# jacobwulffwold/GAN_SR_wind_field

Hardware: AMD Instinct MI355X
Metric: GAN train-steps/sec (G+D fwd+bwd) (higher is better)
Workload: dtype bf16; 1 GPU; C3' full G+D adversarial step: LR 32x32x128 -> HR 128x128x128 (x4), batch 1/GPU, G 16 RRDB nf128 (34.77M), D bf32; preset=C3p, global_batch=1, parallelism=dp1, ranks=1

## Files before the change

### gan_sr_wind_field_amd/csrc/conv_wgrad_tile.hip

```cpp
#include <cstdlib>

#include "common.h"

namespace {

typedef __attribute__((ext_vector_type(4))) short s16x4_t;
typedef s16x4_t __attribute__((address_space(3))) * lds_s16x4_ptr;

struct WgtArgs {
  const unsigned short* x;
  const unsigned short* x2;
  int x2_ctot, x2_c0;
  const unsigned short* dy;
  float* dw;
  const void* zero16;
  int B, Xi, Yi, Zi, Xo, Yo, Zo;
  int Cin, in_ctot, in_off;
  int Cout, out_ctot, out_off;
  int KX, KY, KZ, px, py, pz, ups;
  int TX, TY, TZ;
  int n_chunks, c_chunks, S;
  int tiles_x, tiles_y, tiles_z, ntiles;
  int nbuf;
  int xp_bytes;
  int xs_bytes, buf_bytes;
  int off_buf;
  int tri_base, tri_step;
  int n_active;
  unsigned char act_nc[64], act_cc[64];
  long part_stride;
  int yl_m, yl_ox, yl_oy;
  int xl_m, xl_ox, xl_oy;
  int xl_mz, xl_oz;
  int prio;
  int nphase;
  long class_stride;
  float* bias_parts;
  int S_forced;
  int plan_only;
  unsigned long long* stamps;
  int ablate;
};

__device__ __forceinline__ uint4 tr_frag(const char* lo, const char* hi) {
  s16x4_t a = __builtin_amdgcn_ds_read_tr16_b64_v4i16((lds_s16x4_ptr)(lo));
  s16x4_t b = __builtin_amdgcn_ds_read_tr16_b64_v4i16((lds_s16x4_ptr)(hi));
  uint2 l2 = __builtin_bit_cast(uint2, a), h2 = __builtin_bit_cast(uint2, b);
  return make_uint4(l2.x, l2.y, h2.x, h2.y);
}

__device__ __forceinline__ void glds16(const void* gsrc, unsigned lds_addr) {
  unsigned keep;
  asm volatile(
      "s_mov_b32 %0, m0\n\ts_mov_b32 m0, %2\n\ts_nop 0\n\tglobal_load_lds_dwordx4 %1, off\n\ts_mov_b32 m0, %0"
      : "=&s"(keep)
      : "v"(gsrc), "s"(lds_addr)
      : "memory");
}
__device__ __forceinline__ void dma_wait() { asm volatile("s_waitcnt vmcnt(0)" ::: "memory"); }
__device__ __forceinline__ void dma_wait_upto(int n) {
#define WG_VM(k) case k: asm volatile("s_waitcnt vmcnt(" #k ")" ::: "memory"); break;
  switch (n) {
    WG_VM(0) WG_VM(1) WG_VM(2) WG_VM(3) WG_VM(4) WG_VM(5) WG_VM(6) WG_VM(7) WG_VM(8) WG_VM(9) WG_VM(10) WG_VM(11)
    WG_VM(12) WG_VM(13) WG_VM(14) WG_VM(15) WG_VM(16) WG_VM(17) WG_VM(18) WG_VM(19) WG_VM(20) WG_VM(21) WG_VM(22)
    WG_VM(23) WG_VM(24) WG_VM(25) WG_VM(26) WG_VM(27) WG_VM(28) WG_VM(29) WG_VM(30) WG_VM(31) WG_VM(32) WG_VM(33)
    default: asm volatile("s_waitcnt vmcnt(0)" ::: "memory");
  }
#undef WG_VM
}

#ifdef WSR_CT_STAMPS
#define WG_STAMP(k)                                                                                    \
  do {                                                                                                 \
    if (a.stamps && threadIdx.x == 0) a.stamps[(size_t)blockIdx.x * 8 + (k)] = (k) >= 6 ? clock64() : wall_clock64(); \
  } while (0)
#else
#define WG_STAMP(k) do {} while (0)
#endif

template <int TN> __device__ __forceinline__ int ysw(int v) { return TN == 1 ? 0 : (TN <= 4 ? (v >> 1) & 3 : v & 7); }
constexpr int wgt_rby(int tn) { return tn == 1 ? 32 : (tn <= 4 ? 128 : 256); }

constexpr int wgt_xk(int spw, int tn) { return spw * tn * 4 >= 192 ? 5 : 6; }
constexpr int wgt_yk(int spw, int tn) { return spw * tn * 4 >= 192 ? 4 : 5; }

template <int TN, int SPW, int CT, bool Z16, bool BIAS>
__device__ __forceinline__ void wgrad_tile_body(const WgtArgs& a) {
  static_assert(!BIAS || (TN == 8 && SPW == 1), "one n-tile per wave");
  constexpr int WAVES = 8, NT = 512;
  constexpr int XRPU = 32;
  constexpr int XK = wgt_xk(SPW, TN), YK = wgt_yk(SPW, TN);
  constexpr int RBY = wgt_rby(TN);
  constexpr int YRPU = 1024 / RBY;
  static_assert(TN <= 8, "dy rows hold at most 128 channels");
  extern __shared__ __attribute__((aligned(16))) char smem[];
  const int t = threadIdx.x, lane = t & 63;
  const int wave = __builtin_amdgcn_readfirstlane(t >> 6);
  WG_STAMP(0);
  WG_STAMP(6);

  const int Ly = a.TY + a.KY - 1, Lz = a.TZ + a.KZ - 1, Lx = a.TX + a.KX - 1;
  const int L = Lx * Ly * Lz;
  const int M = a.TX * a.TY * a.TZ;
  const int taps = a.KX * a.KY * a.KZ;
  unsigned short* htab = reinterpret_cast<unsigned short*>(smem);
  char* buf0 = smem + a.off_buf;
  typedef __attribute__((address_space(3))) char* lptr_t;
  const unsigned buf_lds = (unsigned)(unsigned long)(lptr_t)buf0;

  int bid = xcd_remap(blockIdx.x, gridDim.x);
  int cc, nc, s0;
  int cls = 0;
  if (a.nphase == 4) {
    cls = bid & 3;
    bid >>= 2;
  }
  const int px = a.px - (cls >> 1), py = a.py - (cls & 1);
  const int yl_ox = a.nphase == 4 ? (a.yl_m == 2 ? cls >> 1 : 0) : a.yl_ox;
  const int yl_oy = a.nphase == 4 ? (a.yl_m == 2 ? cls & 1 : 0) : a.yl_oy;
  const int xl_ox = a.nphase == 4 ? (a.xl_m == 2 ? px : 0) : a.xl_ox;
  const int xl_oy = a.nphase == 4 ? (a.xl_m == 2 ? py : 0) : a.xl_oy;
  if (a.n_active > 0) {
    const int pr = bid % a.n_active;
    s0 = bid / a.n_active;
    cc = a.act_cc[pr];
    nc = a.act_nc[pr];
  } else {
    cc = bid % a.c_chunks;
    bid /= a.c_chunks;
    nc = bid % a.n_chunks;
    s0 = bid / a.n_chunks;
  }
  const int c0 = cc * 16 * CT, n0 = nc * 16 * TN;
  const bool second = a.x2 != nullptr && c0 >= a.x2_c0;
  const unsigned short* xt = second ? a.x2 : a.x;
  const int x_ctot = second ? a.x2_ctot : a.in_ctot;
  const int x_off = second ? c0 - a.x2_c0 : a.in_off + c0;

  bool act[TN];
  bool any = false;
#pragma unroll
  for (int i = 0; i < TN; ++i) {
    const int n = n0 + 16 * i;
    bool ok = n < a.Cout;
    if (ok && a.tri_step > 0) {
      const int n_last = (n + 15 < a.Cout) ? n + 15 : a.Cout - 1;
      ok = c0 < a.tri_base + a.tri_step * (n_last / a.tri_step);
    }
    act[i] = ok;
    any = any || ok;
  }
  if (!any) return;

  for (int m = t; m < M; m += NT) {
    const int oz = m % a.TZ, r = m / a.TZ;
    const int oy = r % a.TY, ox = r / a.TY;
    htab[m] = (unsigned short)((ox * Ly + oy) * Lz + oz);
  }

  const int U = a.ups ? 1 : 0;
  const int parx = U ? ((-px) & 1) : 0, pary = U ? ((-py) & 1) : 0;
  const int XUP = (L + XRPU - 1) / XRPU;
  const int XU = XUP * CT;
  const int YU = (M + YRPU - 1) / YRPU;
  unsigned xgeo[XK], ygeo[YK];
  int xrel[XK], yrel[YK];
#pragma unroll
  for (int k = 0; k < XK; ++k) {
    const int u = wave + WAVES * k;
    unsigned geo = 0;
    int rel = 0;
    if (u < XU) {
      const int ct = u / XUP;
      const int h = (u - ct * XUP) * XRPU + (lane >> 1);
      const int ch8 = 2 * ct + (lane & 1);
      if (h < L && c0 + 8 * ch8 < a.Cin) {
        const int hz = h % Lz, qq = h / Lz;
        const int hy = qq % Ly, hx = qq / Ly;
        geo = hx | (hy << 8) | (hz << 16) | (1u << 24);
        rel = ((((hx + parx) >> U) * a.xl_m * (a.Yi * a.xl_m) + ((hy + pary) >> U) * a.xl_m) * (a.Zi * a.xl_mz) +
               hz * a.xl_mz) * x_ctot + 8 * ch8;
      }
    }
    xgeo[k] = geo;
    xrel[k] = rel;
  }
#pragma unroll
  for (int k = 0; k < YK; ++k) {
    const int u = wave + WAVES * k;
    unsigned geo = 0;
    int rel = 0;
    if (u < YU) {
      const int v = u * YRPU + lane / (RBY / 16), sl = lane % (RBY / 16);
      const int b32 = (sl >> 1) ^ ysw<TN>(v);
      const int oct = 2 * b32 + (sl & 1);
      if (v < M && b32 < TN && n0 + 8 * oct < a.Cout) {
        const int oz = v % a.TZ, qq = v / a.TZ;
        const int oy = qq % a.TY, ox = qq / a.TY;
        geo = ox | (oy << 8) | (oz << 16) | (1u << 24);
        rel = ((ox * a.yl_m * (a.Yo * a.yl_m) + oy * a.yl_m) * a.Zo + oz) * a.out_ctot + 8 * oct;
      }
    }
    ygeo[k] = geo;
    yrel[k] = rel;
  }

  const unsigned short* zsrc = reinterpret_cast<const unsigned short*>(a.zero16);
  auto issue_tile = [&](int tile, int buf) {
    int r = tile;
    const int tz = r % a.tiles_z; r /= a.tiles_z;
    const int ty = r % a.tiles_y; r /= a.tiles_y;
    const int tx = r % a.tiles_x;
    const int b = r / a.tiles_x;
    const int x0 = tx * a.TX, y0 = ty * a.TY, z0 = tz * a.TZ;
    const unsigned dstx = buf_lds + buf * a.buf_bytes;
    const unsigned dsty = dstx + a.xs_bytes;
    {
      const int lox = px - x0, loy = py - y0, loz = a.pz - z0;
      const int sx_ = a.Xi << U, sy_ = a.Yi << U;
      const bool inner = lox <= 0 && Lx - lox <= sx_ && loy <= 0 && Ly - loy <= sy_ && loz <= 0 && Lz - loz <= a.Zi;
      const long base = ((((long)b * a.Xi * a.xl_m + (long)((x0 - px - parx) >> U) * a.xl_m + xl_ox) * (a.Yi * a.xl_m) +
                          (long)((y0 - py - pary) >> U) * a.xl_m + xl_oy) * (a.Zi * a.xl_mz) +
                         (long)(z0 - a.pz) * a.xl_mz + a.xl_oz) * x_ctot + x_off;
      const unsigned short* bp = xt + base;
#pragma unroll
      for (int k = 0; k < XK; ++k) {
        const int u = wave + WAVES * k;
#ifdef WSR_CT_STAMPS
        if ((a.ablate & 64) && (k & 1)) continue;
        if ((a.ablate & 128) && (k & 3)) continue;
#endif
        if (u < XU) {
          const unsigned geo = xgeo[k];
          bool ok = (geo >> 24) & 1;
          if (!inner)
            ok = ok && (unsigned)((int)(geo & 255) - lox) < (unsigned)sx_ &&
                 (unsigned)((int)((geo >> 8) & 255) - loy) < (unsigned)sy_ &&
                 (unsigned)((int)((geo >> 16) & 255) - loz) < (unsigned)a.Zi;
          glds16(ok ? bp + xrel[k] : zsrc, __builtin_amdgcn_readfirstlane(dstx + u * 1024));
        }
      }
    }
    {
      const int hix = a.Xo - x0, hiy = a.Yo - y0, hiz = a.Zo - z0;
      const bool inner = a.TX <= hix && a.TY <= hiy && a.TZ <= hiz;
      const long base = ((((long)b * a.Xo * a.yl_m + x0 * a.yl_m + yl_ox) * (a.Yo * a.yl_m) + y0 * a.yl_m + yl_oy) *
                             a.Zo + z0) * a.out_ctot + a.out_off + n0;
      const unsigned short* bp = a.dy + base;
#pragma unroll
      for (int k = 0; k < YK; ++k) {
        const int u = wave + WAVES * k;
        if (u < YU) {
          const unsigned geo = ygeo[k];
          bool ok = (geo >> 24) & 1;
          if (!inner)
            ok = ok && (int)(geo & 255) < hix && (int)((geo >> 8) & 255) < hiy && (int)((geo >> 16) & 255) < hiz;
          glds16(ok ? bp + yrel[k] : zsrc, __builtin_amdgcn_readfirstlane(dsty + u * 1024));
        }
      }
    }
  };

  const int nslots = taps * CT;
  int soff[SPW];
#pragma unroll
  for (int j = 0; j < SPW; ++j) {
    const int sj = wave + WAVES * j;
    int off = 0, ct = 0;
    if (sj < nslots) {
      const int tap = sj / CT;
      ct = sj % CT;
      const int kz = tap % a.KZ, r = tap / a.KZ;
      const int ky = r % a.KY, kx = r / a.KY;
      off = (kx * Ly + ky) * Lz + kz;
    }
    soff[j] = __builtin_amdgcn_readfirstlane(off * 32 + ct * a.xp_bytes);
  }

  f32x4_t acc[SPW][TN];
#pragma unroll
  for (int j = 0; j < SPW; ++j)
#pragma unroll
    for (int i = 0; i < TN; ++i) acc[j][i] = f32x4_t{0.f, 0.f, 0.f, 0.f};
  f32x4_t accb = f32x4_t{0.f, 0.f, 0.f, 0.f};

  const int G = lane >> 4, q = (lane & 15) >> 2, p = lane & 3;
  const int ksteps = M >> 5;

  WG_STAMP(1);
#ifdef WSR_CT_STAMPS
  long long st_bar = 0;
  int st_tiles = 0;
#endif
  constexpr bool LEAN = SPW * TN * 4 >= 192;
  constexpr int R = SPW % 7 == 0 ? 7 : (SPW % 4 == 0 ? 4 : (SPW % 3 == 0 ? 3 : 1));
#ifdef WSR_WG_D
  constexpr int D = R > WSR_WG_D ? WSR_WG_D : R - 1;
#else
  constexpr int D = R > 3 ? 3 : R - 1;
#endif
  struct KP { const char *xlo, *xhi, *rlo, *rhi; int slo, shi; };
  auto kp_of = [&](const char* Xs, const char* Ys, int ks) {
    const int m_lo = Z16 ? ks * 32 + 16 * (G >> 1) + 4 * (G & 1) + q : ks * 32 + 4 * G + q;
    const int m_hi = m_lo + (Z16 ? 8 : 16);
    KP k;
    k.xlo = Xs + (int)htab[m_lo] * 32 + p * 8;
    k.rlo = Ys + m_lo * RBY + p * 8;
    k.slo = ysw<TN>(m_lo);
    if constexpr (Z16) {
      k.xhi = k.xlo + 8 * 32;
      k.rhi = k.rlo + 8 * RBY;
      k.shi = k.slo;
    } else {
      k.xhi = Xs + (int)htab[m_hi] * 32 + p * 8;
      k.rhi = Ys + m_hi * RBY + p * 8;
      k.shi = ysw<TN>(m_hi);
    }
    return k;
  };
  constexpr int XHI = 8 * 32, RHI = 8 * RBY;
  auto af_of = [&](const KP& k, int i) {
#ifdef WSR_CT_STAMPS
    if (a.ablate & 4) return make_uint4(lane, 1u, 2u, 3u);
#endif
    if constexpr (Z16) {
      const char* lo = k.rlo + ((i ^ k.slo) << 5);
      return tr_frag(lo, lo + RHI);
    } else {
      return tr_frag(k.rlo + ((i ^ k.slo) << 5), k.rhi + ((i ^ k.shi) << 5));
    }
  };
  auto bf_of = [&](const KP& k, int j) {
#ifdef WSR_CT_STAMPS
    if (a.ablate & 4) return make_uint4(lane, 1u, 2u, 3u);
#endif
    if constexpr (Z16) {
      const char* lo = k.xlo + soff[j];
      return tr_frag(lo, lo + XHI);
    } else {
      return tr_frag(k.xlo + soff[j], k.xhi + soff[j]);
    }
  };

  if (a.prio && wave >= WAVES / 2) __builtin_amdgcn_s_setprio(1);
  const int DT = a.nbuf - 1;
  int upt = 0;
#pragma unroll
  for (int k = 0; k < XK; ++k) upt += (wave + WAVES * k < XU) ? 1 : 0;
#pragma unroll
  for (int k = 0; k < YK; ++k) upt += (wave + WAVES * k < YU) ? 1 : 0;
  const int ntl = (a.ntiles - s0 + a.S - 1) / a.S;
  int bi = 0, bc = 0;
  for (int it = 0;; ++it) {
    const int pre = s0 + it * a.S;
#ifdef WSR_CT_STAMPS
    if (pre < a.ntiles && !((a.ablate & 1) && it > 0)) issue_tile(pre, bi);
#else
    if (pre < a.ntiles) issue_tile(pre, bi);
#endif
    bi = bi + 1 == a.nbuf ? 0 : bi + 1;
    if (it >= DT) {
      const char* Xs = buf0 + bc * a.buf_bytes;
      const char* Ys = Xs + a.xs_bytes;
      bc = bc + 1 == a.nbuf ? 0 : bc + 1;
      if constexpr (LEAN) {
        for (int ks = 0; ks < ksteps; ++ks) {
          const KP k = kp_of(Xs, Ys, ks);
          uint4 af[TN], bfr[2];
#pragma unroll
          for (int i = 0; i < TN; ++i) af[i] = af_of(k, i);
          bfr[0] = bf_of(k, 0);
#pragma unroll
          for (int j = 0; j < SPW; ++j) {
#ifdef WSR_CT_STAMPS
            if ((a.ablate & 16) && ((j + 1) & 3)) { if (j + 1 < SPW) bfr[(j + 1) & 1] = bfr[j & 1]; } else
#endif
            if (j + 1 < SPW) bfr[(j + 1) & 1] = bf_of(k, j + 1);
            __builtin_amdgcn_sched_barrier(0);
#pragma unroll
            for (int i = 0; i < TN; ++i)
              acc[j][i] = __builtin_amdgcn_mfma_f32_16x16x32_bf16(__builtin_bit_cast(bf16x8_t, af[i]),
                                                                  __builtin_bit_cast(bf16x8_t, bfr[j & 1]), acc[j][i], 0, 0, 0);
            __builtin_amdgcn_sched_barrier(0);
          }
        }
      } else {
      KP kc = kp_of(Xs, Ys, 0);
      uint4 afA[TN], afB[TN], ring[R], nb;
#pragma unroll
      for (int i = 0; i < TN; ++i) afA[i] = af_of(kc, i);
#pragma unroll
      for (int d = 0; d < (R > 1 ? D : 1); ++d) ring[d] = bf_of(kc, d);
      auto step = [&](int ks, uint4 (&afc)[TN], uint4 (&afn)[TN]) {
        const KP kn = kp_of(Xs, Ys, ks + 1 < ksteps ? ks + 1 : ks);
        if constexpr (R == 1) nb = bf_of(kn, 0);

#pragma unroll
        for (int j = 0; j < SPW; ++j) {
          if constexpr (R > 1) {
            const int f = j + D;
            if (f < SPW) ring[f % R] = bf_of(kc, f);
            else ring[f % R] = bf_of(kn, f - SPW);
          }
          if (j < TN) afn[j] = af_of(kn, j);
          __builtin_amdgcn_sched_barrier(0);
#ifdef WSR_CT_STAMPS
          if (a.ablate & 8) continue;
#endif
#pragma unroll
          for (int i = 0; i < TN; ++i)
            acc[j][i] = __builtin_amdgcn_mfma_f32_16x16x32_bf16(__builtin_bit_cast(bf16x8_t, afc[i]),
                                                                __builtin_bit_cast(bf16x8_t, ring[j % R]), acc[j][i], 0, 0,
                                                                0);
          __builtin_amdgcn_sched_barrier(0);
        }
        if constexpr (SPW < TN) {
#pragma unroll
          for (int i = SPW; i < TN; ++i) afn[i] = af_of(kn, i);
        }
        if constexpr (BIAS) {
          const uint4 afw = af_of(kc, wave);
          const uint4 ones = make_uint4(0x3F803F80u, 0x3F803F80u, 0x3F803F80u, 0x3F803F80u);
          accb = __builtin_amdgcn_mfma_f32_16x16x32_bf16(__builtin_bit_cast(bf16x8_t, afw), __builtin_bit_cast(bf16x8_t, ones),
                                                         accb, 0, 0, 0);
        }
        if constexpr (R == 1) ring[0] = nb;
        kc = kn;
      };
      for (int ks = 0; ks < ksteps; ks += 2) {
        step(ks, afA, afB);
        if (ks + 1 < ksteps) step(ks + 1, afB, afA);
      }
      }
    }
#ifdef WSR_CT_STAMPS
    const long long tw0 = clock64();
#endif
    {
      const int tnext = it - DT + 1;
      if (tnext >= 0) {
        int later = ntl - 1 - tnext;
        later = later < 0 ? 0 : (later > it - tnext ? it - tnext : later);
        dma_wait_upto(later * upt);
      }
      __syncthreads();
#ifdef WSR_CT_STAMPS
      st_bar += clock64() - tw0;
      ++st_tiles;
#endif
      if (tnext >= 0 && tnext >= ntl) break;
    }
  }
  WG_STAMP(2);

  float* const dwp = a.dw + (long)cls * a.class_stride + (long)s0 * a.part_stride;
  const bool store = a.part_stride > 0;
#pragma unroll
  for (int j = 0; j < SPW; ++j) {
    const int sj = wave + WAVES * j;
    if (sj >= nslots) continue;
    const int tap = sj / CT, ct = sj % CT;
    const int c = c0 + 16 * ct + (lane & 15);
    if (c >= a.Cin) continue;
#pragma unroll
    for (int i = 0; i < TN; ++i) {
      if (!act[i]) continue;
#pragma unroll
      for (int r = 0; r < 4; ++r) {
        const int n = n0 + 16 * i + 4 * G + r;
        if (n < a.Cout) {
          float* q = dwp + ((long)n * taps + tap) * a.Cin + c;
          if (store) *q = acc[j][i][r];
          else atomicAdd(q, acc[j][i][r]);
        }
      }
    }
  }
  if constexpr (BIAS) {
    if (cc == 0 && (lane & 15) == 0) {
#pragma unroll
      for (int r = 0; r < 4; ++r) {
        const int n = n0 + 16 * wave + 4 * G + r;
        if (n < a.Cout) a.bias_parts[(long)s0 * a.Cout + n] = accb[r];
      }
    }
  }
  WG_STAMP(3);
  WG_STAMP(7);
#ifdef WSR_CT_STAMPS
  if (a.stamps && threadIdx.x == 0) {
    a.stamps[(size_t)blockIdx.x * 8 + 4] = (unsigned long long)st_bar;
    a.stamps[(size_t)blockIdx.x * 8 + 5] = (unsigned long long)st_tiles;
  }
#endif
}

template <int TN, int SPW, int CT, bool Z16>
__global__ __launch_bounds__(512) void wgrad_tile_kernel(const WgtArgs a) {
  wgrad_tile_body<TN, SPW, CT, Z16, false>(a);
}
template <bool Z16>
__global__ __launch_bounds__(512) void wgrad_tile_bias_kernel(const WgtArgs a) {
  wgrad_tile_body<8, 1, 8, Z16, true>(a);
}

static inline int round_up(int v, int m) { return (v + m - 1) / m * m; }

__device__ uint4 g_wg_zero16 = {0u, 0u, 0u, 0u};

template <int TN, int SPW, int CT>
int launch_tile(WgtArgs& a, hipStream_t st) {
  constexpr int WAVES = 8;
  const int taps = a.KX * a.KY * a.KZ;
  if (taps * CT > WAVES * SPW) return WSR_EUNSUPPORTED;
  if (a.x2 && a.x2_c0 % (16 * CT)) return WSR_EUNSUPPORTED;
  {
    static void* zp = nullptr;
    if (!zp) {
      hipError_t e = hipGetSymbolAddress(&zp, HIP_SYMBOL(g_wg_zero16));
      if (e != hipSuccess) return (int)e;
    }
    a.zero16 = zp;
  }
  int tz = a.Zo <= 16 ? a.Zo : ((a.Zo % 16 == 0 || a.Zo > 64) ? 16 : 8);
  if (a.KZ == 1 && a.KX * a.KY > 1 && tz > 4 && a.Zo % 4 == 0 && !WSR_ENV_SET("WSR_CT_NOFLAT")) tz = 4;
  static const int cand[][2] = {{8, 8}, {4, 8}, {4, 4}, {2, 4}, {2, 2}, {1, 2}, {1, 1}};
  int best = -1, best_nbuf = 0;
  const int nbuf_want = taps == 1 ? WSR_ENV_INT("WSR_WG_NBUF", 2) : ((SPW == 4 && CT == 1) ? WSR_ENV_INT("WSR_WG_NBUF_THIN", 2) : 2);
  const int mmax = taps == 1 && nbuf_want > 2 ? WSR_ENV_INT("WSR_WG_MMAX", 64) : 1 << 30;
  for (int nbuf = nbuf_want; nbuf >= 2 && best < 0; --nbuf) {
    for (int ci = 0; ci < 7; ++ci) {
      const int tx = cand[ci][0], ty = cand[ci][1];
      const int M = tx * ty * tz;
      if ((M & 31) || M > mmax) continue;
      if (a.ups && ((tx | ty) & 1)) continue;
      const int L = (tx + a.KX - 1) * (ty + a.KY - 1) * (tz + a.KZ - 1);
      const int xs = CT * round_up(L * 32, 1024), ys = round_up(M * wgt_rby(TN), 1024);
      if (xs / 1024 > wgt_xk(SPW, TN) * WAVES || ys / 1024 > wgt_yk(SPW, TN) * WAVES || L > 65535) continue;
      if (round_up(M * 2, 1024) + nbuf * (xs + ys) > 160 * 1024) continue;
      best = ci;
      best_nbuf = nbuf;
      break;
    }
  }
  if (best < 0) return WSR_EUNSUPPORTED;
  a.TX = cand[best][0]; a.TY = cand[best][1]; a.TZ = tz;
  a.nbuf = best_nbuf;
  const int M = a.TX * a.TY * a.TZ;
  const int L = (a.TX + a.KX - 1) * (a.TY + a.KY - 1) * (a.TZ + a.KZ - 1);
  a.xp_bytes = round_up(L * 32, 1024);
  a.xs_bytes = CT * a.xp_bytes;
  a.buf_bytes = a.xs_bytes + round_up(M * wgt_rby(TN), 1024);
  a.off_buf = round_up(M * 2, 1024);
  const size_t lds = (size_t)a.off_buf + (size_t)a.nbuf * a.buf_bytes;
  a.n_chunks = (a.Cout + 16 * TN - 1) / (16 * TN);
  a.c_chunks = (a.Cin + 16 * CT - 1) / (16 * CT);
  a.tiles_x = (a.Xo + a.TX - 1) / a.TX;
  a.tiles_y = (a.Yo + a.TY - 1) / a.TY;
  a.tiles_z = (a.Zo + a.TZ - 1) / a.TZ;
  a.ntiles = a.B * a.tiles_x * a.tiles_y * a.tiles_z;
  int combos = a.n_chunks * a.c_chunks;
  a.n_active = 0;
  if (a.tri_step > 0 && combos <= 64) {
    for (int nc = 0; nc < a.n_chunks; ++nc)
      for (int cc = 0; cc < a.c_chunks; ++cc) {
        bool any = false;
        for (int i = 0; i < TN; ++i) {
          const int n = nc * 16 * TN + 16 * i;
          if (n >= a.Cout) continue;
          const int n_last = (n + 15 < a.Cout) ? n + 15 : a.Cout - 1;
          any = any || cc * 16 * CT < a.tri_base + a.tri_step * (n_last / a.tri_step);
        }
        if (any) {
          a.act_nc[a.n_active] = (unsigned char)nc;
          a.act_cc[a.n_active] = (unsigned char)cc;
          ++a.n_active;
        }
      }
    if (a.n_active == 0) { a.S = 0; return 0; }
    combos = a.n_active;
  }
  const int nphase = a.nphase == 4 ? 4 : 1;
  int S = 256 / (combos * nphase);
  if (S < 1) {
    if (nphase > 1) return WSR_EUNSUPPORTED;
    S = 1;
  }
  if (S > a.ntiles) S = a.ntiles;
  a.S = S;
  if (WSR_ENV_SET("WSR_WGRAD_S")) {
    const int v = WSR_ENV_RAW("WSR_WGRAD_S");
    if (v >= 1 && v <= a.ntiles) a.S = v;
  }
  if (a.plan_only) return 0;
  if (a.part_stride > 0 && a.S_forced != a.S) return WSR_EINVAL;
  const bool z16 = a.TZ % 16 == 0;
  auto kern = z16 ? wgrad_tile_kernel<TN, SPW, CT, true> : wgrad_tile_kernel<TN, SPW, CT, false>;
  int ki = z16;
  if (a.bias_parts) {
    if constexpr (TN == 8 && SPW == 1) {
      kern = z16 ? wgrad_tile_bias_kernel<true> : wgrad_tile_bias_kernel<false>;
      ki += 2;
    } else {
      return WSR_EUNSUPPORTED;
    }
  }
  static bool attr_done[4] = {false, false, false, false};
  if (!attr_done[ki]) {
    hipError_t e = hipFuncSetAttribute(reinterpret_cast<const void*>(kern), hipFuncAttributeMaxDynamicSharedMemorySize,
                                       160 * 1024);
    if (e != hipSuccess) return (int)e;
    attr_done[ki] = true;
  }
#ifdef WSR_CT_STAMPS
  a.stamps = getenv("WSR_CT_STAMPS_PTR") ? (unsigned long long*)strtoull(getenv("WSR_CT_STAMPS_PTR"), nullptr, 0) : nullptr;
  a.ablate = WSR_ENV_INT("WSR_CT_ABL", 0);
#endif
  a.prio = WSR_ENV_INT("WSR_CT_PRIO", 0);
  hipLaunchKernelGGL(kern, dim3((unsigned)(combos * a.S * nphase)), dim3(WAVES * 64), lds, st, a);
  WSR_LAUNCH_CHECK();
  return 0;
}

}

namespace {
int run_tile(WgtArgs& a, int taps, int Cout, int Cin, hipStream_t st);
}

static int wgrad_tile_bf16_any(const wsr_conv_t* c, const void* x, const void* dy, float* dw, int tri_base, int tri_step,
                               long part_stride, int n_parts, int* plan, void* stream, const void* x2, int x2_ctot,
                               int x2_c0, long class_stride, float* bias_parts = nullptr, bool want_bias = false);

int wsr_wgrad_tile_bf16(const wsr_conv_t* c, const void* x, const void* dy, float* dw, int tri_base, int tri_step,
                        long part_stride, int n_parts, int* plan, void* stream, const void* x2, int x2_ctot, int x2_c0) {
  return wgrad_tile_bf16_any(c, x, dy, dw, tri_base, tri_step, part_stride, n_parts, plan, stream, x2, x2_ctot, x2_c0, 0);
}

int wsr_wgrad_tile_bf16_lat4(const wsr_conv_t* c, const void* x, const void* dy, float* parts, long part_stride,
                             long class_stride, int n_parts, int* plan, void* stream) {
  if ((c->lat != 2 && c->lat != 3) || c->lat_ox || c->lat_oy || c->px < 1 || c->py < 1) return WSR_EUNSUPPORTED;
  if (c->lat == 3 && (c->px != 1 || c->py != 1)) return WSR_EUNSUPPORTED;
  if (c->lat == 2 && c->lat_mz > 1) return WSR_EUNSUPPORTED;
  return wgrad_tile_bf16_any(c, x, dy, parts, 0, 0, part_stride, n_parts, plan, stream, nullptr, 0, 0, class_stride);
}

int wsr_wgrad_tile_bf16_bias(const wsr_conv_t* c, const void* x, const void* dy, float* parts, long part_stride, int n_parts,
                             float* bias_parts, int* plan, void* stream) {
  return wgrad_tile_bf16_any(c, x, dy, parts, 0, 0, part_stride, n_parts, plan, stream, nullptr, 0, 0, 0, bias_parts, true);
}

static int wgrad_tile_bf16_any(const wsr_conv_t* c, const void* x, const void* dy, float* dw, int tri_base, int tri_step,
                               long part_stride, int n_parts, int* plan, void* stream, const void* x2, int x2_ctot,
                               int x2_c0, long class_stride, float* bias_parts, bool want_bias) {
  if (want_bias && (c->KX * c->KY * c->KZ != 1 || c->lat || c->upsample_xy || c->Cout < 64 || c->Cin < 64 || x2 || tri_step > 0))
    return WSR_EUNSUPPORTED;
  if (c->dtype != WSR_BF16 || (c->sx | c->sy | c->sz) != 1) return WSR_EUNSUPPORTED;
  if (x2 && (c->lat || c->upsample_xy || tri_step > 0 || x2_c0 <= 0 || x2_c0 >= c->Cin || x2_c0 % 32 || x2_ctot % 8 ||
             c->Cin - x2_c0 > x2_ctot))
    return WSR_EUNSUPPORTED;
  if (c->lat == 2 && (c->lat_phases || c->lat_mz > 1 || tri_step > 0)) return WSR_EUNSUPPORTED;
  if (c->lat == 3 && (c->lat_phases || tri_step > 0 || c->upsample_xy)) return WSR_EUNSUPPORTED;
  const int taps = c->KX * c->KY * c->KZ;
  if (taps > 128) return WSR_EUNSUPPORTED;
  if (c->Cin % 8 || c->in_ctot % 8 || c->in_off % 8 || c->out_ctot % 8 || c->out_off % 8) return WSR_EUNSUPPORTED;
  if (c->out_off + (c->Cout + 7) / 8 * 8 > c->out_ctot) return WSR_EUNSUPPORTED;
  if (c->KX > 8 || c->KY > 8 || c->KZ > 8) return WSR_EUNSUPPORTED;
  WgtArgs a{};
  a.x = (const unsigned short*)x;
  a.x2 = (const unsigned short*)x2; a.x2_ctot = x2_ctot; a.x2_c0 = x2_c0;
  a.dy = (const unsigned short*)dy;
  a.dw = dw;
  a.B = c->B; a.Xi = c->Xi; a.Yi = c->Yi; a.Zi = c->Zi;
  a.Xo = c->Xo; a.Yo = c->Yo; a.Zo = c->Zo;
  a.Cin = c->Cin; a.in_ctot = c->in_ctot; a.in_off = c->in_off;
  a.Cout = c->Cout; a.out_ctot = c->out_ctot; a.out_off = c->out_off;
  a.KX = c->KX; a.KY = c->KY; a.KZ = c->KZ;
  a.px = c->px; a.py = c->py; a.pz = c->pz;
  a.ups = c->upsample_xy ? 1 : 0;
  a.yl_m = c->lat == 2 ? 2 : 1; a.yl_ox = c->lat == 2 ? c->lat_ox : 0; a.yl_oy = c->lat == 2 ? c->lat_oy : 0;
  a.xl_m = a.xl_mz = 1;
  if (c->lat == 3) {
    a.xl_m = 2; a.xl_ox = c->lat_ox; a.xl_oy = c->lat_oy;
    a.xl_mz = c->lat_mz > 1 ? c->lat_mz : 1; a.xl_oz = c->lat_oz;
  }
  a.tri_base = tri_base; a.tri_step = tri_step;
  a.part_stride = part_stride; a.S_forced = n_parts; a.plan_only = plan ? 1 : 0;
  a.bias_parts = bias_parts;
  a.nphase = class_stride != 0 ? 4 : 1;
  a.class_stride = class_stride > 0 ? class_stride : 0;
  if (taps == 1 && !c->lat && !c->upsample_xy && c->Zi % 16 != 0 && (c->px | c->py | c->pz) == 0) {
    const long nv = (long)c->Xi * c->Yi * c->Zi;
    if (nv % 128 == 0 && nv / 128 < (1L << 24)) {
      a.Xi = a.Xo = (int)(nv / 128);
      a.Yi = a.Yo = 8;
      a.Zi = a.Zo = 16;
    }
  }
  hipStream_t st = as_stream(stream);
  const int rc = run_tile(a, taps, c->Cout, c->Cin, st);
  if (plan && rc == 0) *plan = a.S;
  return rc;
}

namespace {
int run_tile(WgtArgs& a, int taps, int Cout, int Cin, hipStream_t st) {
  struct { int Cout, Cin; } cc{Cout, Cin};
  auto* c = &cc;
  if (taps == 1) {
    if (c->Cout < 64 || c->Cin < 64) return WSR_EUNSUPPORTED;
    return launch_tile<8, 1, 8>(a, st);
  }
  if (taps > 28) {
    if (c->Cout <= 16) return launch_tile<1, 16, 1>(a, st);
    if (c->Cout % 48 == 0) return launch_tile<3, 16, 1>(a, st);
    return launch_tile<2, 16, 1>(a, st);
  }
  if (taps <= 12 && c->Cout >= 64 && c->Cin >= 64) {
    const int rc = launch_tile<4, 6, 4>(a, st);
    if (rc != WSR_EUNSUPPORTED) return rc;
  }
  const bool small = a.tri_step == 0 && !WSR_ENV_SET("WSR_WG_NOSMALL");
  if (small && taps <= 12 && c->Cout > 16 && c->Cout <= 32) {
    const int rc = launch_tile<2, 3, 2>(a, st);
    if (rc != WSR_EUNSUPPORTED) return rc;
  }
  if (small && c->Cin <= 16 && c->Cout <= 32) {
    const int rc = c->Cout <= 16 ? launch_tile<1, 4, 1>(a, st) : launch_tile<2, 4, 1>(a, st);
    if (rc != WSR_EUNSUPPORTED) return rc;
  }
  if (c->Cin <= 16 && c->Cout % 48 == 0 && a.tri_step == 0 && !WSR_ENV_SET("WSR_WG_NO341")) {
    const int rc = launch_tile<3, 4, 1>(a, st);
    if (rc != WSR_EUNSUPPORTED) return rc;
  }
  if (c->Cout <= 16) return launch_tile<1, 7, 2>(a, st);
  if (c->Cout <= 32) return launch_tile<2, 7, 2>(a, st);
  return launch_tile<4, 7, 2>(a, st);
}
}
```

Measured before the change: 11.61 train-steps/s.

## Spread wgrad tile DMA issue across MFMA k-steps with incremental tile addressing

Once the prologue is done, the weight-gradient tile kernel no longer issues all global-to-LDS loads for the next tile in one burst. It spreads them over the MFMA k-steps a few units at a time, so memory issue overlaps compute. Tile base offsets are now advanced incrementally instead of recomputed with div/mod. Per-unit geometry is packed into compact vectors with 5-bit coordinates. This assumes tile extents below 32 and adds scheduling barriers inside the MFMA loop. The old burst behaviour is still available through an environment variable.

```diff
diff --git a/gan_sr_wind_field_amd/csrc/conv_wgrad_tile.hip b/gan_sr_wind_field_amd/csrc/conv_wgrad_tile.hip
--- a/gan_sr_wind_field_amd/csrc/conv_wgrad_tile.hip
+++ b/gan_sr_wind_field_amd/csrc/conv_wgrad_tile.hip
@@ -40,6 +40,7 @@
   int plan_only;
   unsigned long long* stamps;
   int ablate;
+  int burst;
 };
 
 __device__ __forceinline__ uint4 tr_frag(const char* lo, const char* hi) {
@@ -163,102 +164,137 @@
   const int XUP = (L + XRPU - 1) / XRPU;
   const int XU = XUP * CT;
   const int YU = (M + YRPU - 1) / YRPU;
-  unsigned xgeo[XK], ygeo[YK];
-  int xrel[XK], yrel[YK];
-#pragma unroll
-  for (int k = 0; k < XK; ++k) {
-    const int u = wave + WAVES * k;
+  constexpr int NK = XK + YK;
+  typedef int relv_t __attribute__((ext_vector_type(NK)));
+  typedef unsigned geov_t __attribute__((ext_vector_type((NK + 1) / 2)));
+  int nxo_ = 0, nyo_ = 0;
+#pragma unroll
+  for (int k = 0; k < XK; ++k) nxo_ += (wave + WAVES * k < XU) ? 1 : 0;
+#pragma unroll
+  for (int k = 0; k < YK; ++k) nyo_ += (wave + WAVES * k < YU) ? 1 : 0;
+  const int nxo = __builtin_amdgcn_readfirstlane(nxo_), nyo = __builtin_amdgcn_readfirstlane(nyo_);
+  const int upt = nxo + nyo;
+  relv_t relv;
+  geov_t geov;
+#pragma unroll
+  for (int j = 0; j < NK; ++j) {
+    int rel = -1;
     unsigned geo = 0;
-    int rel = 0;
-    if (u < XU) {
+    if (j < nxo) {
+      const int u = wave + WAVES * j;
       const int ct = u / XUP;
       const int h = (u - ct * XUP) * XRPU + (lane >> 1);
       const int ch8 = 2 * ct + (lane & 1);
       if (h < L && c0 + 8 * ch8 < a.Cin) {
         const int hz = h % Lz, qq = h / Lz;
         const int hy = qq % Ly, hx = qq / Ly;
-        geo = hx | (hy << 8) | (hz << 16) | (1u << 24);
+        geo = hx | (hy << 5) | (hz << 10);
         rel = ((((hx + parx) >> U) * a.xl_m * (a.Yi * a.xl_m) + ((hy + pary) >> U) * a.xl_m) * (a.Zi * a.xl_mz) +
                hz * a.xl_mz) * x_ctot + 8 * ch8;
       }
-    }
-    xgeo[k] = geo;
-    xrel[k] = rel;
-  }
-#pragma unroll
-  for (int k = 0; k < YK; ++k) {
-    const int u = wave + WAVES * k;
-    unsigned geo = 0;
-    int rel = 0;
-    if (u < YU) {
+    } else if (j < upt) {
+      const int u = wave + WAVES * (j - nxo);
       const int v = u * YRPU + lane / (RBY / 16), sl = lane % (RBY / 16);
       const int b32 = (sl >> 1) ^ ysw<TN>(v);
       const int oct = 2 * b32 + (sl & 1);
       if (v < M && b32 < TN && n0 + 8 * oct < a.Cout) {
         const int oz = v % a.TZ, qq = v / a.TZ;
         const int oy = qq % a.TY, ox = qq / a.TY;
-        geo = ox | (oy << 8) | (oz << 16) | (1u << 24);
+        geo = ox | (oy << 5) | (oz << 10);
         rel = ((ox * a.yl_m * (a.Yo * a.yl_m) + oy * a.yl_m) * a.Zo + oz) * a.out_ctot + 8 * oct;
       }
     }
-    ygeo[k] = geo;
-    yrel[k] = rel;
+    relv[j] = rel;
+    if (j & 1) geov[j >> 1] |= geo << 16;
+    else geov[j >> 1] = geo;
+  }
+
+  const int sx_ = a.Xi << U, sy_ = a.Yi << U, zi_ = a.Zi;
+  auto xbase_of = [&](int b, int tx, int ty, int tz) {
+    const int x0 = tx * a.TX, y0 = ty * a.TY, z0 = tz * a.TZ;
+    return ((((long)b * a.Xi * a.xl_m + (long)((x0 - px - parx) >> U) * a.xl_m + xl_ox) * (a.Yi * a.xl_m) +
+             (long)((y0 - py - pary) >> U) * a.xl_m + xl_oy) * (a.Zi * a.xl_mz) +
+            (long)(z0 - a.pz) * a.xl_mz + a.xl_oz) * x_ctot + x_off;
+  };
+  auto ybase_of = [&](int b, int tx, int ty, int tz) {
+    const int x0 = tx * a.TX, y0 = ty * a.TY, z0 = tz * a.TZ;
+    return ((((long)b * a.Xo * a.yl_m + x0 * a.yl_m + yl_ox) * (a.Yo * a.yl_m) + y0 * a.yl_m + yl_oy) *
+                a.Zo + z0) * a.out_ctot + a.out_off + n0;
+  };
+  int t_z, t_y, t_x, t_b, d_z, d_y, d_x, d_b;
+  {
+    int r = s0;
+    t_z = r % a.tiles_z; r /= a.tiles_z;
+    t_y = r % a.tiles_y; r /= a.tiles_y;
+    t_x = r % a.tiles_x; t_b = r / a.tiles_x;
+    r = a.S;
+    d_z = r % a.tiles_z; r /= a.tiles_z;
+    d_y = r % a.tiles_y; r /= a.tiles_y;
+    d_x = r % a.tiles_x; d_b = r / a.tiles_x;
+  }
+  long offx = xbase_of(t_b, t_x, t_y, t_z), offy = ybase_of(t_b, t_x, t_y, t_z);
+  long stx, cxz, cxy, cxx, sty, cyz, cyy, cyx;
+  {
+    const long x0_ = xbase_of(0, 0, 0, 0), xz = xbase_of(0, 0, 0, 1) - x0_, xy = xbase_of(0, 0, 1, 0) - x0_,
+               xx = xbase_of(0, 1, 0, 0) - x0_, xb = xbase_of(1, 0, 0, 0) - x0_;
+    stx = d_b * xb + d_x * xx + d_y * xy + d_z * xz;
+    cxz = xy - a.tiles_z * xz; cxy = xx - a.tiles_y * xy; cxx = xb - a.tiles_x * xx;
+    const long y0_ = ybase_of(0, 0, 0, 0), yz = ybase_of(0, 0, 0, 1) - y0_, yy = ybase_of(0, 0, 1, 0) - y0_,
+               yx = ybase_of(0, 1, 0, 0) - y0_, yb = ybase_of(1, 0, 0, 0) - y0_;
+    sty = d_b * yb + d_x * yx + d_y * yy + d_z * yz;
+    cyz = yy - a.tiles_z * yz; cyy = yx - a.tiles_y * yy; cyx = yb - a.tiles_x * yx;
   }
 
   const unsigned short* zsrc = reinterpret_cast<const unsigned short*>(a.zero16);
-  auto issue_tile = [&](int tile, int buf) {
-    int r = tile;
-    const int tz = r % a.tiles_z; r /= a.tiles_z;
-    const int ty = r % a.tiles_y; r /= a.tiles_y;
-    const int tx = r % a.tiles_x;
-    const int b = r / a.tiles_x;
-    const int x0 = tx * a.TX, y0 = ty * a.TY, z0 = tz * a.TZ;
-    const unsigned dstx = buf_lds + buf * a.buf_bytes;
-    const unsigned dsty = dstx + a.xs_bytes;
-    {
-      const int lox = px - x0, loy = py - y0, loz = a.pz - z0;
-      const int sx_ = a.Xi << U, sy_ = a.Yi << U;
-      const bool inner = lox <= 0 && Lx - lox <= sx_ && loy <= 0 && Ly - loy <= sy_ && loz <= 0 && Lz - loz <= a.Zi;
-      const long base = ((((long)b * a.Xi * a.xl_m + (long)((x0 - px - parx) >> U) * a.xl_m + xl_ox) * (a.Yi * a.xl_m) +
-                          (long)((y0 - py - pary) >> U) * a.xl_m + xl_oy) * (a.Zi * a.xl_mz) +
-                         (long)(z0 - a.pz) * a.xl_mz + a.xl_oz) * x_ctot + x_off;
-      const unsigned short* bp = xt + base;
-#pragma unroll
-      for (int k = 0; k < XK; ++k) {
-        const int u = wave + WAVES * k;
-#ifdef WSR_CT_STAMPS
-        if ((a.ablate & 64) && (k & 1)) continue;
-        if ((a.ablate & 128) && (k & 3)) continue;
-#endif
-        if (u < XU) {
-          const unsigned geo = xgeo[k];
-          bool ok = (geo >> 24) & 1;
-          if (!inner)
-            ok = ok && (unsigned)((int)(geo & 255) - lox) < (unsigned)sx_ &&
-                 (unsigned)((int)((geo >> 8) & 255) - loy) < (unsigned)sy_ &&
-                 (unsigned)((int)((geo >> 16) & 255) - loz) < (unsigned)a.Zi;
-          glds16(ok ? bp + xrel[k] : zsrc, __builtin_amdgcn_readfirstlane(dstx + u * 1024));
-        }
-      }
-    }
-    {
-      const int hix = a.Xo - x0, hiy = a.Yo - y0, hiz = a.Zo - z0;
-      const bool inner = a.TX <= hix && a.TY <= hiy && a.TZ <= hiz;
-      const long base = ((((long)b * a.Xo * a.yl_m + x0 * a.yl_m + yl_ox) * (a.Yo * a.yl_m) + y0 * a.yl_m + yl_oy) *
-                             a.Zo + z0) * a.out_ctot + a.out_off + n0;
-      const unsigned short* bp = a.dy + base;
-#pragma unroll
-      for (int k = 0; k < YK; ++k) {
-        const int u = wave + WAVES * k;
-        if (u < YU) {
-          const unsigned geo = ygeo[k];
-          bool ok = (geo >> 24) & 1;
-          if (!inner)
-            ok = ok && (int)(geo & 255) < hix && (int)((geo >> 8) & 255) < hiy && (int)((geo >> 16) & 255) < hiz;
-          glds16(ok ? bp + yrel[k] : zsrc, __builtin_amdgcn_readfirstlane(dsty + u * 1024));
-        }
-      }
-    }
+  const unsigned short *bpx = xt, *bpy = a.dy;
+  unsigned dst0 = 0;
+  int lox = 0, loy = 0, loz = 0;
+  int hix = 0, hiy = 0, hiz = 0;
+  int tin = 1;
+  const unsigned ydst = (unsigned)(a.xs_bytes - nxo * (WAVES * 1024));
+  auto next_tile = [&](int buf) {
+    const int x0 = t_x * a.TX, y0 = t_y * a.TY, z0 = t_z * a.TZ;
+    lox = px - x0; loy = py - y0; loz = a.pz - z0;
+    hix = a.Xo - x0; hiy = a.Yo - y0; hiz = a.Zo - z0;
+    tin = (lox <= 0 && Lx - lox <= sx_ && loy <= 0 && Ly - loy <= sy_ && loz <= 0 && Lz - loz <= a.Zi && a.TX <= hix &&
+           a.TY <= hiy && a.TZ <= hiz) ? 1 : 0;
+    bpx = xt + offx;
+    bpy = a.dy + offy;
+    dst0 = buf_lds + buf * a.buf_bytes + wave * 1024;
+    offx += stx; offy += sty;
+    t_z += d_z;
+    if (t_z >= a.tiles_z) { t_z -= a.tiles_z; ++t_y; offx += cxz; offy += cyz; }
+    t_y += d_y;
+    if (t_y >= a.tiles_y) { t_y -= a.tiles_y; ++t_x; offx += cxy; offy += cyy; }
+    t_x += d_x;
+    if (t_x >= a.tiles_x) { t_x -= a.tiles_x; ++t_b; offx += cxx; offy += cyx; }
+    t_b += d_b;
+  };
+  auto unit = [&](int j, bool inner) __attribute__((always_inline)) {
+    const bool isy = j >= nxo;
+#ifdef WSR_CT_STAMPS
+    if (!isy && (((a.ablate & 64) && (j & 1)) || ((a.ablate & 128) && (j & 3)))) return;
+#endif
+    const int rel = relv[j];
+    int ok = rel >= 0 ? 1 : 0;
+    if (!inner) {
+      const unsigned geo = geov[j >> 1] >> ((j & 1) << 4);
+      const int lx = isy ? 0 : lox, ly = isy ? 0 : loy, lz = isy ? 0 : loz;
+      const unsigned ex = isy ? hix : sx_, ey = isy ? hiy : sy_, ez = isy ? hiz : zi_;
+      ok &= ((unsigned)((int)(geo & 31) - lx) < ex ? 1 : 0) & ((unsigned)((int)((geo >> 5) & 31) - ly) < ey ? 1 : 0) &
+            ((unsigned)((int)((geo >> 10) & 31) - lz) < ez ? 1 : 0);
+    }
+    const unsigned short* bp = isy ? bpy : bpx;
+    glds16(ok ? bp + rel : zsrc, __builtin_amdgcn_readfirstlane(dst0 + j * (WAVES * 1024) + (isy ? ydst : 0u)));
+  };
+  auto issue_units = [&](int j, int j1) __attribute__((always_inline)) {
+    __builtin_amdgcn_sched_barrier(0);
+    if (tin) {
+      for (; j < j1; ++j) unit(j, true);
+    } else {
+      for (; j < j1; ++j) unit(j, false);
+    }
+    __builtin_amdgcn_sched_barrier(0);
   };
 
   const int nslots = taps * CT;
@@ -344,20 +380,20 @@
 
   if (a.prio && wave >= WAVES / 2) __builtin_amdgcn_s_setprio(1);
   const int DT = a.nbuf - 1;
-  int upt = 0;
-#pragma unroll
-  for (int k = 0; k < XK; ++k) upt += (wave + WAVES * k < XU) ? 1 : 0;
-#pragma unroll
-  for (int k = 0; k < YK; ++k) upt += (wave + WAVES * k < YU) ? 1 : 0;
   const int ntl = (a.ntiles - s0 + a.S - 1) / a.S;
+  const int per = (upt + ksteps - 1) / ksteps;
   int bi = 0, bc = 0;
   for (int it = 0;; ++it) {
-    const int pre = s0 + it * a.S;
-#ifdef WSR_CT_STAMPS
-    if (pre < a.ntiles && !((a.ablate & 1) && it > 0)) issue_tile(pre, bi);
+    int jc = 0, jn = 0;
+#ifdef WSR_CT_STAMPS
+    if (it < ntl && !((a.ablate & 1) && it > 0)) {
 #else
-    if (pre < a.ntiles) issue_tile(pre, bi);
-#endif
+    if (it < ntl) {
+#endif
+      next_tile(bi);
+      if (it < DT || a.burst) issue_units(0, upt);
+      else jn = upt;
+    }
     bi = bi + 1 == a.nbuf ? 0 : bi + 1;
     if (it >= DT) {
       const char* Xs = buf0 + bc * a.buf_bytes;
@@ -383,6 +419,9 @@
                                                                   __builtin_bit_cast(bf16x8_t, bfr[j & 1]), acc[j][i], 0, 0, 0);
             __builtin_amdgcn_sched_barrier(0);
           }
+          const int j1 = jc + per < jn ? jc + per : jn;
+          issue_units(jc, j1);
+          jc = j1;
         }
       } else {
       KP kc = kp_of(Xs, Ys, 0);
@@ -426,6 +465,9 @@
         }
         if constexpr (R == 1) ring[0] = nb;
         kc = kn;
+        const int j1 = jc + per < jn ? jc + per : jn;
+        issue_units(jc, j1);
+        jc = j1;
       };
       for (int ks = 0; ks < ksteps; ks += 2) {
         step(ks, afA, afB);
@@ -617,6 +659,7 @@
   a.ablate = WSR_ENV_INT("WSR_CT_ABL", 0);
 #endif
   a.prio = WSR_ENV_INT("WSR_CT_PRIO", 0);
+  a.burst = WSR_ENV_INT("WSR_WG_DMA_BURST", 0) ? 1 : 0;
   hipLaunchKernelGGL(kern, dim3((unsigned)(combos * a.S * nphase)), dim3(WAVES * 64), lds, st, a);
   WSR_LAUNCH_CHECK();
   return 0;
```

New measurement: 11.68 train-steps/s (median of 6 runs). About the same (+0.6%).
